# MARSLab-UMN/vi_depth_completion

Hardware: AMD Instinct MI355X
Metric: frames/sec (higher is better)
Workload: dtype f32

## Files before the change

### vi_depth_completion_amd/csrc/wfused.hip

```cpp
#include "common.h"
#include <cstdlib>

#pragma clang fp contract(off)

namespace {

typedef float f32x4 __attribute__((ext_vector_type(4)));

constexpr int TB = 16, NBW = 32, KC = 16, NPOS = 36;
constexpr int NPW = 8, NTW = 8, NTHREADS = 64 * (NPW + NTW);
constexpr int VBUF = NPOS * TB * KC;
constexpr int XSLOT = 37;
constexpr int XBUF = TB * XSLOT * KC;
constexpr int NDMA = TB * XSLOT / 16;
constexpr int MLD = 36;
constexpr size_t LDS_BYTES = (size_t)(2 * VBUF + 2 * XBUF) * sizeof(float);
static_assert(TB * XSLOT % 16 == 0, "whole DMA instructions");
static_assert((size_t)NPOS * TB * MLD * sizeof(float) <= LDS_BYTES, "the epilogue's product rows reuse the buffers");
static_assert(LDS_BYTES <= 160 * 1024, "one workgroup per CU");

struct FArgs {
    const float* x; const float* u; float* y; const float* s1; const float* b1; const float* s2; const float* b2;
    int H, W, Cin, ldx, Cout, ldy, th, tw, T, flags, nbn, gn;
    long long x_gs, w_gs, y_gs, p_gs;
    unsigned x_bytes;
};

typedef __attribute__((address_space(3))) void lds_void_t;

template <typename V> __device__ __forceinline__ void bt6_lo(const V (&d)[6], V (&t)[3]) {
    const V p = d[4] - 4.f * d[2], q = d[3] - 4.f * d[1];
    t[0] = (4.f * d[0] - 5.f * d[2]) + d[4];
    t[1] = p + q;
    t[2] = p - q;
}
template <typename V> __device__ __forceinline__ void bt6_hi(const V (&d)[6], V (&t)[3]) {
    const V r = d[4] - d[2], s = 2.f * (d[3] - d[1]);
    t[0] = r + s;
    t[1] = r - s;
    t[2] = (4.f * d[1] - 5.f * d[3]) + d[5];
}
template <typename V> __device__ __forceinline__ void bt6(const V (&d)[6], V (&t)[6]) {
    V lo[3], hi[3];
    bt6_lo(d, lo);
    bt6_hi(d, hi);
#pragma unroll
    for (int i = 0; i < 3; ++i) { t[i] = lo[i]; t[3 + i] = hi[i]; }
}
__device__ __forceinline__ void at6(const float (&m)[6], float (&o)[4]) {
    const float s12 = m[1] + m[2], d12 = m[1] - m[2], s34 = m[3] + m[4], d34 = m[3] - m[4];
    o[0] = (m[0] + s12) + s34;
    o[1] = d12 + 2.f * d34;
    o[2] = s12 + 4.f * s34;
    o[3] = (d12 + 8.f * d34) + m[5];
}

template <int N_> __device__ __forceinline__ void wait_lgkmcnt() { asm volatile("s_waitcnt lgkmcnt(%0)" ::"n"(N_) : "memory"); }
__device__ __forceinline__ f32x4 lds_read_b128(unsigned addr) {
    f32x4 v;
    asm volatile("ds_read_b128 %0, %1" : "=v"(v) : "v"(addr));
    return v;
}
template <int OFF> __device__ __forceinline__ float lds_read_b32(unsigned addr) {
    float v;
    asm volatile("ds_read_b32 %0, %1 offset:%2" : "=v"(v) : "v"(addr), "n"(OFF));
    return v;
}
template <int OFF> __device__ __forceinline__ void lds_write_b32(unsigned addr, float v) { asm volatile("ds_write_b32 %0, %1 offset:%2" ::"v"(addr), "v"(v), "n"(OFF) : "memory"); }

template <int PW, int NB, int DBG>
__device__ __forceinline__ void product_wave(const FArgs& a, float* smem, unsigned lds0, int lane, int pos0, int g, int nb, int NK) {
    const int n = lane & 15, kq = lane >> 4;
    const int n32 = a.Cout / 32, pair = NB == 2 ? nb : nb >> 1, half = NB == 2 ? 0 : nb & 1;
    const float* ub = a.u + (size_t)g * a.w_gs + ((size_t)pos0 * n32 + pair) * ((size_t)NK * 512) + half * 256 + lane * 4;
    const size_t pos_stride = (size_t)n32 * NK * 512;
    auto load_b = [&](int p, int kc, f32x4 (&dst)[NB]) {
        const float* s = ub + (size_t)p * pos_stride + (size_t)kc * 512;
        dst[0] = *reinterpret_cast<const f32x4*>(s);
        if constexpr (NB == 2) dst[1] = *reinterpret_cast<const f32x4*>(s + 256);
    };
    f32x4 acc[PW][NB];
#pragma unroll
    for (int p = 0; p < PW; ++p)
#pragma unroll
        for (int j = 0; j < NB; ++j) acc[p][j] = f32x4{0.f, 0.f, 0.f, 0.f};
    f32x4 bq[PW][NB];
#pragma unroll
    for (int p = 0; p < PW; ++p) load_b(p, 0, bq[p]);
    const unsigned a_off = (unsigned)((n * KC + ((kq ^ ((n >> 2) & 3)) * 4)) * 4);
    const unsigned a_wave = lds0 + (unsigned)(pos0 * TB * KC * 4);

    __builtin_amdgcn_s_barrier();
    __builtin_amdgcn_s_barrier();
    __builtin_amdgcn_s_barrier();
    for (int kc = 0; kc < NK; ++kc) {
        const unsigned vb = a_wave + (unsigned)((kc & 1) * VBUF * 4);
        const int kn = kc + 1 < NK ? kc + 1 : kc;
        f32x4 fa[2];
        fa[0] = lds_read_b128(vb + a_off);
#pragma unroll
        for (int p = 0; p < PW; ++p) {
            const int cur = p & 1, nxt = cur ^ 1;
            if (p + 1 < PW) {
                fa[nxt] = lds_read_b128(vb + (unsigned)((p + 1) * TB * KC * 4) + a_off);
                wait_lgkmcnt<1>();
            } else {
                wait_lgkmcnt<0>();
            }
            __builtin_amdgcn_sched_barrier(0);
#pragma unroll
            for (int ks = 0; ks < 4; ++ks)
#pragma unroll
                for (int j = 0; j < NB; ++j)
                    if constexpr (!(DBG & 1)) acc[p][j] = __builtin_amdgcn_mfma_f32_16x16x4f32(fa[cur][ks], bq[p][j][ks], acc[p][j], 0, 0, 0);
                    else if (ks == 0) acc[p][j][0] += fa[cur][0] + fa[cur][3] + bq[p][j][0] + bq[p][j][3];
            if constexpr (!(DBG & 2)) load_b(p, kn, bq[p]);
            __builtin_amdgcn_sched_barrier(0);
        }
        __builtin_amdgcn_s_barrier();
    }
    asm volatile("s_waitcnt vmcnt(0)" ::: "memory");
    float* mx = smem;
#pragma unroll
    for (int p = 0; p < PW; ++p)
#pragma unroll
        for (int j = 0; j < NB; ++j)
#pragma unroll
            for (int i = 0; i < 4; ++i) mx[((pos0 + p) * TB + 4 * kq + i) * MLD + j * 16 + n] = acc[p][j][i];
}

template <int NB, int DBG>
__global__ void __launch_bounds__(NTHREADS)
wino4_fused_kernel(const FArgs a) {
    extern __shared__ __attribute__((aligned(16))) float smem[];
    const int tid = threadIdx.x;
    const int L = blockIdx.x;
    const int tb = L / a.gn, r_ = L - tb * a.gn, g = r_ / a.nbn, nb = r_ - g * a.nbn;
    const int NK = a.Cin / KC;
    const unsigned lds0 = (unsigned)(size_t)((__attribute__((address_space(3))) float*)smem);

    if (tid < 64 * NPW) {
        const int w = __builtin_amdgcn_readfirstlane(tid >> 6);
        if (w < 4) product_wave<5, NB, DBG>(a, smem, lds0, tid & 63, 5 * w, g, nb, NK);
        else product_wave<4, NB, DBG>(a, smem, lds0, tid & 63, 20 + 4 * (w - 4), g, nb, NK);
    } else {
        const int tt = tid - 64 * NPW, lane = tid & 63;
        const int w8 = __builtin_amdgcn_readfirstlane(tt >> 6), grp = w8 >> 2;
        const int u_ = tt & 255, m = u_ >> 4, c = u_ & 15;
        const int tpf = a.th * a.tw;
        constexpr unsigned OOB = 0x80000000u;
        unsigned voff[5];
#pragma unroll
        for (int i = 0; i < 5; ++i) {
            const int j = w8 + 8 * i;
            const int slot = 16 * j + (lane >> 2), quad = lane & 3;
            const int ts = slot / XSLOT, px = slot - ts * XSLOT;
            const int t = tb * TB + ts;
            bool ok = j < NDMA && px < 36 && t < a.T;
            const int tc = ok ? t : 0;
            const int b = tc / tpf, rem = tc - b * tpf, ty = rem / a.tw, tx = rem - ty * a.tw;
            const int r = px / 6, s = px - r * 6;
            const int iy = ty * 4 - 1 + r, ix = tx * 4 - 1 + s;
            ok = ok && (unsigned)iy < (unsigned)a.H && (unsigned)ix < (unsigned)a.W;
            voff[i] = ok ? (unsigned)(((size_t)((b * a.H + iy) * a.W + ix) * a.ldx + (size_t)g * a.x_gs + quad * 4) * 4) : OOB;
        }
        const __amdgpu_buffer_rsrc_t x_rsrc = __builtin_amdgcn_make_buffer_rsrc(const_cast<float*>(a.x), 0, (int)a.x_bytes, 0x00020000);
        auto dma = [&](int cc) {
            float* dst = smem + 2 * VBUF + (cc & 1) * XBUF;
            const int soff = cc * KC * 4;
#pragma unroll
            for (int i = 0; i < 5; ++i)
                if (w8 + 8 * i < NDMA) __builtin_amdgcn_raw_ptr_buffer_load_lds(x_rsrc, (lds_void_t*)(dst + (w8 + 8 * i) * 256), 16, (int)voff[i], soff, 0, 0);
        };
        float out[36];
        const unsigned x_thr = lds0 + (unsigned)((2 * VBUF + (m * XSLOT) * KC + c) * 4);
        const unsigned v_thr = lds0 + (unsigned)((m * KC + (((c >> 2) ^ ((m >> 2) & 3)) * 4) + (c & 3)) * 4);
        auto phase_a = [&](int cc) {
            const unsigned xa = x_thr + (unsigned)((cc & 1) * XBUF * 4);
            float D[36];
#define VIDC_RD(i) D[i] = lds_read_b32<(i) * KC * 4>(xa);
            VIDC_RD(0) VIDC_RD(1) VIDC_RD(2) VIDC_RD(3) VIDC_RD(4) VIDC_RD(5) VIDC_RD(6) VIDC_RD(7) VIDC_RD(8) VIDC_RD(9) VIDC_RD(10) VIDC_RD(11)
            VIDC_RD(12) VIDC_RD(13) VIDC_RD(14) VIDC_RD(15) VIDC_RD(16) VIDC_RD(17) VIDC_RD(18) VIDC_RD(19) VIDC_RD(20) VIDC_RD(21) VIDC_RD(22) VIDC_RD(23)
            VIDC_RD(24) VIDC_RD(25) VIDC_RD(26) VIDC_RD(27) VIDC_RD(28) VIDC_RD(29) VIDC_RD(30) VIDC_RD(31) VIDC_RD(32) VIDC_RD(33) VIDC_RD(34) VIDC_RD(35)
#undef VIDC_RD
            asm volatile("s_waitcnt lgkmcnt(0)" : "+v"(D[0]), "+v"(D[1]), "+v"(D[2]), "+v"(D[3]), "+v"(D[4]), "+v"(D[5]), "+v"(D[6]), "+v"(D[7]), "+v"(D[8]), "+v"(D[9]), "+v"(D[10]), "+v"(D[11]), "+v"(D[12]), "+v"(D[13]), "+v"(D[14]), "+v"(D[15]), "+v"(D[16]), "+v"(D[17]) :: "memory");
            asm volatile("" : "+v"(D[18]), "+v"(D[19]), "+v"(D[20]), "+v"(D[21]), "+v"(D[22]), "+v"(D[23]), "+v"(D[24]), "+v"(D[25]), "+v"(D[26]), "+v"(D[27]), "+v"(D[28]), "+v"(D[29]), "+v"(D[30]), "+v"(D[31]), "+v"(D[32]), "+v"(D[33]), "+v"(D[34]), "+v"(D[35]) :: "memory");
            float tcol[6][6];
#pragma unroll
            for (int s = 0; s < 6; ++s) {
                float col[6], o6[6];
#pragma unroll
                for (int r = 0; r < 6; ++r) col[r] = D[r * 6 + s];
                bt6(col, o6);
#pragma unroll
                for (int r = 0; r < 6; ++r) tcol[r][s] = o6[r];
            }
#pragma unroll
            for (int r = 0; r < 6; ++r) {
                float o6[6];
                bt6(tcol[r], o6);
#pragma unroll
                for (int s = 0; s < 6; ++s) out[r * 6 + s] = o6[s];
            }
        };
        auto phase_b = [&](int cc) {
            const unsigned va = v_thr + (unsigned)((cc & 1) * VBUF * 4);
#define VIDC_WR(i) lds_write_b32<(i) * TB * KC * 4>(va, out[i]);
            VIDC_WR(0) VIDC_WR(1) VIDC_WR(2) VIDC_WR(3) VIDC_WR(4) VIDC_WR(5) VIDC_WR(6) VIDC_WR(7) VIDC_WR(8) VIDC_WR(9) VIDC_WR(10) VIDC_WR(11)
            VIDC_WR(12) VIDC_WR(13) VIDC_WR(14) VIDC_WR(15) VIDC_WR(16) VIDC_WR(17) VIDC_WR(18) VIDC_WR(19) VIDC_WR(20) VIDC_WR(21) VIDC_WR(22) VIDC_WR(23)
            VIDC_WR(24) VIDC_WR(25) VIDC_WR(26) VIDC_WR(27) VIDC_WR(28) VIDC_WR(29) VIDC_WR(30) VIDC_WR(31) VIDC_WR(32) VIDC_WR(33) VIDC_WR(34) VIDC_WR(35)
#undef VIDC_WR
        };
        auto fence_barrier = [&]() {
            if constexpr (DBG & 16) asm volatile("s_waitcnt lgkmcnt(0)" ::: "memory");
            else asm volatile("s_waitcnt vmcnt(0) lgkmcnt(0)" ::: "memory");
            __builtin_amdgcn_s_barrier();
        };
        dma(0);
        if (NK > 1) dma(1);
        fence_barrier();
        if (grp == 0) phase_a(0);
        else if (NK > 1) phase_a(1);
        fence_barrier();
        if (NK > 2) dma(2);
        if (grp == 0) phase_b(0);
        fence_barrier();
        for (int it = 0; it < NK; ++it) {
            if (!(DBG & 4)) {
                if (it + 3 < NK) dma(it + 3);
                if ((it & 1) == grp) {
                    if (it + 2 < NK) phase_a(it + 2);
                } else {
                    if (it + 1 < NK) phase_b(it + 1);
                }
            }
            fence_barrier();
        }
    }
    __syncthreads();
    if (tid < TB * 16 * NB) {
        const int m = tid / (16 * NB), c = tid - m * (16 * NB);
        const int t = tb * TB + m;
        if (t >= a.T || (DBG & 8)) return;
        const int tpf = a.th * a.tw;
        const int b = t / tpf, rem = t - b * tpf, ty = rem / a.tw, tx = rem - ty * a.tw;
        const float* mx = smem + m * MLD + c;
        float tc[4][6];
#pragma unroll
        for (int s = 0; s < 6; ++s) {
            float col[6], o4[4];
#pragma unroll
            for (int r = 0; r < 6; ++r) col[r] = mx[(r * 6 + s) * TB * MLD];
            at6(col, o4);
#pragma unroll
            for (int r = 0; r < 4; ++r) tc[r][s] = o4[r];
        }
        const int ch = nb * 16 * NB + c;
        const float s1 = a.s1[(size_t)g * a.p_gs + ch], b1 = a.b1[(size_t)g * a.p_gs + ch];
        const bool aff2 = a.flags & VIDC_AFFINE2;
        const float s2 = aff2 ? a.s2[(size_t)g * a.p_gs + ch] : 0.f, b2 = aff2 ? a.b2[(size_t)g * a.p_gs + ch] : 0.f;
        const float lo1 = (a.flags & VIDC_RELU1) ? 0.f : -INFINITY, lo2 = (a.flags & VIDC_RELU2) ? 0.f : -INFINITY;
        float* yb = a.y + (size_t)g * a.y_gs + ch;
#pragma unroll
        for (int r = 0; r < 4; ++r) {
            float o4[4];
            at6(tc[r], o4);
            const int oy = ty * 4 + r;
            if (oy >= a.H) continue;
#pragma unroll
            for (int s = 0; s < 4; ++s) {
                const int ox = tx * 4 + s;
                if (ox >= a.W) continue;
                float o = fmaxf(o4[s] * s1 + b1, lo1);
                if (aff2) o = fmaxf(o * s2 + b2, lo2);
                yb[((size_t)(b * a.H + oy) * a.W + ox) * a.ldy] = o;
            }
        }
    }
}

__global__ void __launch_bounds__(256)
wino4_pack_kernel(const float* __restrict__ u, float* __restrict__ o, int Cout, int Cin, long long total4) {
    const long long i = (long long)blockIdx.x * blockDim.x + threadIdx.x;
    if (i >= total4) return;
    const int NK = Cin / KC, nbn = Cout / NBW;
    const int lane = (int)(i & 63), nblk = (int)((i >> 6) & 1);
    long long r = i >> 7;
    const int kc = (int)(r % NK); r /= NK;
    const int nb = (int)(r % nbn);
    const int pos = (int)(r / nbn);
    const int n = lane & 15, kq = lane >> 4;
    const float4 v = *reinterpret_cast<const float4*>(u + ((size_t)pos * Cout + nb * NBW + nblk * 16 + n) * Cin + kc * KC + kq * 4);
    *reinterpret_cast<float4*>(o + i * 4) = v;
}

template <int NB, int DBG>
int launch_nb(const FArgs& a, long long wgs, hipStream_t st) {
    static bool attr_set[64] = {};
    int dev = 0;
    VIDC_HIP(hipGetDevice(&dev));
    if (dev < 0 || dev >= 64 || !attr_set[dev]) {
        VIDC_HIP(hipFuncSetAttribute(reinterpret_cast<const void*>(&wino4_fused_kernel<NB, DBG>), hipFuncAttributeMaxDynamicSharedMemorySize, (int)LDS_BYTES));
        if (dev >= 0 && dev < 64) attr_set[dev] = true;
    }
    hipLaunchKernelGGL((wino4_fused_kernel<NB, DBG>), dim3((unsigned)wgs), dim3(NTHREADS), LDS_BYTES, st, a);
    VIDC_CHECK_LAUNCH("wino4_fused_kernel");
    return VIDC_OK;
}

template <int DBG>
int launch_dbg(const FArgs& a, long long wgs, hipStream_t st) { return a.nbn * 32 == a.Cout ? launch_nb<2, DBG>(a, wgs, st) : launch_nb<1, DBG>(a, wgs, st); }

}

namespace vidc {

int launch_wino4_fused(const vidc_conv_desc& d, hipStream_t st) {
    VIDC_REQUIRE(d.precision == VIDC_PREC_FP32, VIDC_ERR_SHAPE, "conv (fused Winograd): fp32 arithmetic only");
    VIDC_REQUIRE(d.KH == 3 && d.KW == 3 && d.stride == 1 && d.pad == 1 && d.dilation <= 1, VIDC_ERR_SHAPE, "conv (fused Winograd): 3x3 / stride 1 / pad 1 / dense only");
    VIDC_REQUIRE(d.Cin % KC == 0 && d.Cout % NBW == 0 && d.ldx % 4 == 0, VIDC_ERR_SHAPE, "conv (fused Winograd): Cin %% 16 == 0, Cout %% 32 == 0, ldx %% 4 == 0");
    VIDC_REQUIRE(!(d.flags & ~(VIDC_RELU1 | VIDC_AFFINE2 | VIDC_RELU2)), VIDC_ERR_SHAPE, "conv (fused Winograd): flags 0x%x not supported (affine / ReLU / second affine / ReLU only)", d.flags);
    VIDC_REQUIRE(d.w_gs == (long long)NPOS * d.Cout * d.Cin || d.groups == 1, VIDC_ERR_SHAPE, "conv (fused Winograd): w = U of vidc_winograd_weight_pack_fused, w_gs = 36 * Cout * Cin");
    VIDC_REQUIRE((reinterpret_cast<uintptr_t>(d.x) & 15) == 0 && (reinterpret_cast<uintptr_t>(d.w) & 15) == 0 && d.x_gs % 4 == 0, VIDC_ERR_SHAPE, "conv (fused Winograd): x and U 16-byte aligned");
    FArgs a;
    a.x = d.x; a.u = d.w; a.y = d.y; a.s1 = d.scale1; a.b1 = d.shift1; a.s2 = d.scale2; a.b2 = d.shift2;
    a.H = d.H; a.W = d.W; a.Cin = d.Cin; a.ldx = d.ldx; a.Cout = d.Cout; a.ldy = d.ldy;
    a.th = (d.H + 3) / 4; a.tw = (d.W + 3) / 4;
    a.T = d.B * a.th * a.tw;
    static const int force_nb = [] { const char* e = getenv("VIDC_WFUSED_NB"); return e ? atoi(e) : 0; }();
    const long long wgs32 = (long long)((d.B * a.th * a.tw + TB - 1) / TB) * d.groups * (d.Cout / NBW);
    const int nbk = force_nb == 1 || force_nb == 2 ? force_nb : (wgs32 * 2 <= 256 ? 1 : 2);
    a.flags = d.flags; a.nbn = d.Cout / (16 * nbk); a.gn = d.groups * a.nbn;
    a.x_gs = d.x_gs; a.w_gs = d.w_gs; a.y_gs = d.y_gs; a.p_gs = d.p_gs;
    VIDC_REQUIRE((long long)d.B * d.H * d.W * d.ldx * 4 < (1ll << 30), VIDC_ERR_SHAPE, "conv (fused Winograd): the input must stay below 1 GiB");
    a.x_bytes = (unsigned)((long long)d.B * d.H * d.W * d.ldx * 4);
    const long long wgs = (long long)((a.T + TB - 1) / TB) * a.gn;
    VIDC_REQUIRE(wgs < (1ll << 31), VIDC_ERR_SHAPE, "conv (fused Winograd): grid too large");
#ifdef VIDC_WFUSED_ATTRIB
    static const int dbg = [] { const char* e = getenv("VIDC_WFUSED_DBG"); return e ? atoi(e) : 0; }();
    switch (dbg) {
        case 1: return launch_dbg<1>(a, wgs, st);
        case 2: return launch_dbg<2>(a, wgs, st);
        case 4: return launch_dbg<4>(a, wgs, st);
        case 8: return launch_dbg<8>(a, wgs, st);
        case 3: return launch_dbg<3>(a, wgs, st);
        case 6: return launch_dbg<6>(a, wgs, st);
        case 7: return launch_dbg<7>(a, wgs, st);
        case 15: return launch_dbg<15>(a, wgs, st);
        case 16: return launch_dbg<16>(a, wgs, st);
        default: break;
    }
#endif
    return launch_dbg<0>(a, wgs, st);
}

}

extern "C" int vidc_winograd_weight_pack_fused(const float* u, float* u_packed, int Cout, int Cin, vidc_stream_t stream) {
    VIDC_REQUIRE(u && u_packed && u != u_packed, VIDC_ERR_NULL, "vidc_winograd_weight_pack_fused: null pointer (or in place)");
    VIDC_REQUIRE(Cout > 0 && Cin > 0 && Cout % NBW == 0 && Cin % KC == 0, VIDC_ERR_SHAPE, "vidc_winograd_weight_pack_fused: Cout must be a multiple of 32, Cin of 16");
    const long long total4 = (long long)NPOS * Cout * Cin / 4;
    hipLaunchKernelGGL(wino4_pack_kernel, dim3((unsigned)((total4 + 255) / 256)), dim3(256), 0, vidc::as_stream(stream), u, u_packed, Cout, Cin, total4);
    VIDC_CHECK_LAUNCH("wino4_pack_kernel");
    return VIDC_OK;
}
```

Measured before the change: 635.3.

## Add persistent Winograd kernel specialised for Cin=64 convolutions

Adds a persistent-grid Winograd F(4,3) kernel used whenever Cin is 64. Each workgroup holds all 64 input channels' weights in registers and keeps them across work items that share the same output-channel block. It prefetches the next tile's input patch during the epilogue and uses buffer loads and stores for bounds handling. The goal is to avoid reloading weights per tile and to cut launch/grid overhead for these layers. In exchange it raises register pressure and ties the grid size to the CU count.

```diff
diff --git a/vi_depth_completion_amd/csrc/wfused.hip b/vi_depth_completion_amd/csrc/wfused.hip
--- a/vi_depth_completion_amd/csrc/wfused.hip
+++ b/vi_depth_completion_amd/csrc/wfused.hip
@@ -24,6 +24,8 @@
     int H, W, Cin, ldx, Cout, ldy, th, tw, T, flags, nbn, gn;
     long long x_gs, w_gs, y_gs, p_gs;
     unsigned x_bytes;
+    int items;
+    unsigned y_bytes;
 };
 
 typedef __attribute__((address_space(3))) void lds_void_t;
@@ -279,6 +281,169 @@
     }
 }
 
+constexpr int SK = 64, SNK = SK / KC, SWAVES = 8, STHREADS = 64 * SWAVES, SPW = NPOS * 2 / SWAVES;
+constexpr int SVB = NPOS * SNK * TB * KC;
+constexpr size_t S_LDS_BYTES = (size_t)SVB * sizeof(float);
+static_assert(SPW * SWAVES == NPOS * 2, "whole positions per wave");
+static_assert(NPOS * TB * MLD <= SVB, "the product rows reuse V");
+static_assert(S_LDS_BYTES <= 160 * 1024, "one workgroup per CU");
+static_assert(STHREADS == TB * NBW, "fold: one thread per (tile, channel)");
+static_assert(SNK * (TB / 4) == 2 * SWAVES, "transform: two passes of (chunk, four tiles) per wave");
+
+template <int DBG>
+__global__ void __launch_bounds__(STHREADS)
+wino4_stem_kernel(const FArgs a) {
+    extern __shared__ __attribute__((aligned(16))) float smem[];
+    const int tid = threadIdx.x, lane = tid & 63;
+    const int w = __builtin_amdgcn_readfirstlane(tid >> 6);
+    const int nwg = (int)gridDim.x;
+    int L = (int)blockIdx.x;
+    if ((nwg & 7) == 0) L = (L & 7) * (nwg >> 3) + (L >> 3);
+    const int n32 = a.nbn, tpf = a.th * a.tw;
+    const int n = lane & 15, kq = lane >> 4;
+    const int jb = w & 1, pos0 = SPW * (w >> 1);
+    constexpr unsigned OOB_ROW = 0x80000000u, OOB_COL = 0x40000000u;
+    const __amdgpu_buffer_rsrc_t x_rsrc = __builtin_amdgcn_make_buffer_rsrc(const_cast<float*>(a.x), 0, (int)a.x_bytes, 0x00020000);
+    const __amdgpu_buffer_rsrc_t y_rsrc = __builtin_amdgcn_make_buffer_rsrc(a.y, 0, (int)a.y_bytes, 0x00020000);
+    const int a_off = n * KC + ((kq ^ ((n >> 2) & 3)) * 4);
+    auto load_patch = [&](int tb, int g, int pass, float (&D)[36]) {
+        const int q = pass * SWAVES + w, kc = q & 3, m = (q >> 2) * 4 + (lane >> 4), c16 = lane & 15;
+        const int t = tb * TB + m;
+        const bool tok = t < a.T;
+        const int tc = tok ? t : 0;
+        const int b = tc / tpf, rem = tc - b * tpf, ty = rem / a.tw, tx = rem - ty * a.tw;
+        unsigned rowo[6], colo[6];
+#pragma unroll
+        for (int r = 0; r < 6; ++r) {
+            const int iy = ty * 4 - 1 + r, ix = tx * 4 - 1 + r;
+            rowo[r] = tok && (unsigned)iy < (unsigned)a.H ? (unsigned)((b * a.H + iy) * a.W) * (unsigned)a.ldx * 4u : OOB_ROW;
+            colo[r] = (unsigned)ix < (unsigned)a.W ? (unsigned)(((size_t)ix * a.ldx + (size_t)g * a.x_gs + kc * KC + c16) * 4) : OOB_COL;
+        }
+#pragma unroll
+        for (int r = 0; r < 6; ++r)
+#pragma unroll
+            for (int s = 0; s < 6; ++s)
+                if constexpr (!(DBG & 2)) D[r * 6 + s] = __builtin_bit_cast(float, __builtin_amdgcn_raw_buffer_load_b32(x_rsrc, (int)(rowo[r] + colo[s]), 0, 0));
+                else D[r * 6 + s] = __builtin_bit_cast(float, rowo[r] + colo[s]);
+    };
+    auto col_step = [&](const float (&D)[36], float (&tcol)[6][6]) {
+#pragma unroll
+        for (int s = 0; s < 6; ++s) {
+            float col[6], o6[6];
+#pragma unroll
+            for (int r = 0; r < 6; ++r) col[r] = D[r * 6 + s];
+            bt6(col, o6);
+#pragma unroll
+            for (int r = 0; r < 6; ++r) tcol[r][s] = o6[r];
+        }
+    };
+    auto row_step = [&](const float (&tcol)[6][6], int pass) {
+        const int q = pass * SWAVES + w, kc = q & 3, m = (q >> 2) * 4 + (lane >> 4), c16 = lane & 15;
+        float* vw = smem + (kc * TB + m) * KC + (((c16 >> 2) ^ ((m >> 2) & 3)) * 4) + (c16 & 3);
+#pragma unroll
+        for (int r = 0; r < 6; ++r) {
+            float o6[6];
+            bt6(tcol[r], o6);
+#pragma unroll
+            for (int s = 0; s < 6; ++s) vw[(r * 6 + s) * (SNK * TB * KC)] = o6[s];
+        }
+    };
+    const int fm = tid >> 5, fc = tid & 31;
+    f32x4 U[SPW][SNK];
+    float s1 = 0.f, b1 = 0.f, s2 = 0.f, b2 = 0.f;
+    const bool aff2 = a.flags & VIDC_AFFINE2;
+    const float lo1 = (a.flags & VIDC_RELU1) ? 0.f : -INFINITY, lo2 = (a.flags & VIDC_RELU2) ? 0.f : -INFINITY;
+    int cur = -1;
+    float D[36];
+    if constexpr (!(DBG & 4))
+        if (L < a.items) load_patch(L / a.gn, (L % a.gn) / n32, 0, D);
+    for (int item = L; item < a.items; item += nwg) {
+        const int tb = item / a.gn, combo = item - tb * a.gn, g = combo / n32, pair = combo - g * n32;
+        if (combo != cur) {
+            cur = combo;
+            const float* ub = a.u + (size_t)g * a.w_gs + ((size_t)pos0 * n32 + pair) * (size_t)(SNK * 512) + jb * 256 + lane * 4;
+#pragma unroll
+            for (int u = 0; u < SPW; ++u)
+#pragma unroll
+                for (int kc = 0; kc < SNK; ++kc) U[u][kc] = *reinterpret_cast<const f32x4*>(ub + (size_t)u * n32 * (SNK * 512) + kc * 512);
+            const size_t pc = (size_t)g * a.p_gs + pair * NBW + fc;
+            s1 = a.s1[pc]; b1 = a.b1[pc];
+            if (aff2) { s2 = a.s2[pc]; b2 = a.b2[pc]; }
+        }
+        if constexpr (!(DBG & 4)) {
+            float tcol[6][6];
+            col_step(D, tcol);
+            load_patch(tb, g, 1, D);
+            row_step(tcol, 0);
+            col_step(D, tcol);
+            row_step(tcol, 1);
+        }
+        __syncthreads();
+        f32x4 acc[SPW];
+#pragma unroll
+        for (int u = 0; u < SPW; ++u) acc[u] = f32x4{0.f, 0.f, 0.f, 0.f};
+        const float* va = smem + pos0 * (SNK * TB * KC) + a_off;
+#pragma unroll
+        for (int kc = 0; kc < SNK; ++kc) {
+            f32x4 fa[SPW];
+#pragma unroll
+            for (int u = 0; u < SPW; ++u) fa[u] = *reinterpret_cast<const f32x4*>(va + (u * SNK + kc) * (TB * KC));
+#pragma unroll
+            for (int ks = 0; ks < 4; ++ks)
+#pragma unroll
+                for (int u = 0; u < SPW; ++u)
+                    if constexpr (!(DBG & 1)) acc[u] = __builtin_amdgcn_mfma_f32_16x16x4f32(fa[u][ks], U[u][kc][ks], acc[u], 0, 0, 0);
+                    else if (ks == 0) acc[u][0] += fa[u][0] + fa[u][3] + U[u][kc][0] + U[u][kc][3];
+        }
+        __syncthreads();
+#pragma unroll
+        for (int u = 0; u < SPW; ++u)
+#pragma unroll
+            for (int i = 0; i < 4; ++i) smem[((pos0 + u) * TB + 4 * kq + i) * MLD + jb * 16 + n] = acc[u][i];
+        __syncthreads();
+        if constexpr (!(DBG & 4)) {
+            const int nxt = item + nwg < a.items ? item + nwg : item;
+            load_patch(nxt / a.gn, (nxt % a.gn) / n32, 0, D);
+        }
+        if constexpr (!(DBG & 8)) {
+            const int t = tb * TB + fm;
+            const bool tok = t < a.T;
+            const int tc = tok ? t : 0;
+            const int b = tc / tpf, rem = tc - b * tpf, ty = rem / a.tw, tx = rem - ty * a.tw;
+            unsigned rowo[4], colo[4];
+#pragma unroll
+            for (int r = 0; r < 4; ++r) {
+                const int oy = ty * 4 + r, ox = tx * 4 + r;
+                rowo[r] = tok && oy < a.H ? (unsigned)((b * a.H + oy) * a.W) * (unsigned)a.ldy * 4u : OOB_ROW;
+                colo[r] = ox < a.W ? (unsigned)(((size_t)ox * a.ldy + (size_t)g * a.y_gs + pair * NBW + fc) * 4) : OOB_COL;
+            }
+            const float* mx = smem + fm * MLD + fc;
+            float tc4[4][6];
+#pragma unroll
+            for (int s = 0; s < 6; ++s) {
+                float col[6], o4[4];
+#pragma unroll
+                for (int r = 0; r < 6; ++r) col[r] = mx[(r * 6 + s) * TB * MLD];
+                at6(col, o4);
+#pragma unroll
+                for (int r = 0; r < 4; ++r) tc4[r][s] = o4[r];
+            }
+#pragma unroll
+            for (int r = 0; r < 4; ++r) {
+                float o4[4];
+                at6(tc4[r], o4);
+#pragma unroll
+                for (int s = 0; s < 4; ++s) {
+                    float o = fmaxf(o4[s] * s1 + b1, lo1);
+                    if (aff2) o = fmaxf(o * s2 + b2, lo2);
+                    __builtin_amdgcn_raw_buffer_store_b32(__builtin_bit_cast(unsigned, o), y_rsrc, (int)(rowo[r] + colo[s]), 0, 0);
+                }
+            }
+        }
+        __syncthreads();
+    }
+}
+
 __global__ void __launch_bounds__(256)
 wino4_pack_kernel(const float* __restrict__ u, float* __restrict__ o, int Cout, int Cin, long long total4) {
     const long long i = (long long)blockIdx.x * blockDim.x + threadIdx.x;
@@ -310,6 +475,59 @@
 
 template <int DBG>
 int launch_dbg(const FArgs& a, long long wgs, hipStream_t st) { return a.nbn * 32 == a.Cout ? launch_nb<2, DBG>(a, wgs, st) : launch_nb<1, DBG>(a, wgs, st); }
+
+template <int DBG>
+int launch_stem_dbg(const FArgs& a, long long wgs, hipStream_t st) {
+    static bool attr_set[64] = {};
+    int dev = 0;
+    VIDC_HIP(hipGetDevice(&dev));
+    if (dev < 0 || dev >= 64 || !attr_set[dev]) {
+        VIDC_HIP(hipFuncSetAttribute(reinterpret_cast<const void*>(&wino4_stem_kernel<DBG>), hipFuncAttributeMaxDynamicSharedMemorySize, (int)S_LDS_BYTES));
+        if (dev >= 0 && dev < 64) attr_set[dev] = true;
+    }
+    hipLaunchKernelGGL(wino4_stem_kernel<DBG>, dim3((unsigned)wgs), dim3(STHREADS), S_LDS_BYTES, st, a);
+    VIDC_CHECK_LAUNCH("wino4_stem_kernel");
+    return VIDC_OK;
+}
+
+int launch_stem(FArgs& a, const vidc_conv_desc& d, hipStream_t st) {
+    static int n_cu[64] = {};
+    int dev = 0;
+    VIDC_HIP(hipGetDevice(&dev));
+    const bool cached = dev >= 0 && dev < 64;
+    int cus = cached ? n_cu[dev] : 0;
+    if (cus <= 0) {
+        VIDC_HIP(hipDeviceGetAttribute(&cus, hipDeviceAttributeMultiprocessorCount, dev));
+        VIDC_REQUIRE(cus > 0, VIDC_ERR_SHAPE, "conv (fused Winograd): no compute units");
+        if (cached) n_cu[dev] = cus;
+    }
+    a.nbn = d.Cout / NBW; a.gn = d.groups * a.nbn;
+    const long long y_bytes = ((long long)(d.groups - 1) * d.y_gs + ((long long)d.B * d.H * d.W - 1) * d.ldy + d.Cout) * 4;
+    VIDC_REQUIRE(d.y_gs >= 0 && d.ldy > 0 && y_bytes < (1ll << 30), VIDC_ERR_SHAPE, "conv (fused Winograd, Cin = 64): the output must stay below 1 GiB");
+    a.y_bytes = (unsigned)y_bytes;
+    const long long items = (long long)((a.T + TB - 1) / TB) * a.gn;
+    VIDC_REQUIRE(items > 0 && items < (1ll << 30), VIDC_ERR_SHAPE, "conv (fused Winograd): grid too large");
+    a.items = (int)items;
+    const char* e = getenv("VIDC_WFUSED_WGS");
+    const int forced = e ? atoi(e) : 0;
+    long long wgs = forced > 0 ? forced : (a.gn <= cus ? (long long)(cus / a.gn) * a.gn : cus);
+    if (wgs > items) wgs = items;
+#ifdef VIDC_WFUSED_ATTRIB
+    static const int dbg = [] { const char* v = getenv("VIDC_WFUSED_DBG"); return v ? atoi(v) : 0; }();
+    switch (dbg) {
+        case 1: return launch_stem_dbg<1>(a, wgs, st);
+        case 2: return launch_stem_dbg<2>(a, wgs, st);
+        case 4: return launch_stem_dbg<4>(a, wgs, st);
+        case 8: return launch_stem_dbg<8>(a, wgs, st);
+        case 3: return launch_stem_dbg<3>(a, wgs, st);
+        case 5: return launch_stem_dbg<5>(a, wgs, st);
+        case 12: return launch_stem_dbg<12>(a, wgs, st);
+        case 13: return launch_stem_dbg<13>(a, wgs, st);
+        default: break;
+    }
+#endif
+    return launch_stem_dbg<0>(a, wgs, st);
+}
 
 }
 
@@ -334,7 +552,9 @@
     a.x_gs = d.x_gs; a.w_gs = d.w_gs; a.y_gs = d.y_gs; a.p_gs = d.p_gs;
     VIDC_REQUIRE((long long)d.B * d.H * d.W * d.ldx * 4 < (1ll << 30), VIDC_ERR_SHAPE, "conv (fused Winograd): the input must stay below 1 GiB");
     a.x_bytes = (unsigned)((long long)d.B * d.H * d.W * d.ldx * 4);
-    const long long wgs = (long long)((a.T + TB - 1) / TB) * a.gn;
+    a.items = 0;
+    if (d.Cin == SK) return launch_stem(a, d, st);
+    const long long wgs =(long long)((a.T + TB - 1) / TB) * a.gn;
     VIDC_REQUIRE(wgs < (1ll << 31), VIDC_ERR_SHAPE, "conv (fused Winograd): grid too large");
 #ifdef VIDC_WFUSED_ATTRIB
     static const int dbg = [] { const char* e = getenv("VIDC_WFUSED_DBG"); return e ? atoi(e) : 0; }();
```

Result: no change. 636.0 (median of 2 runs) (+0.1%).

## Add persistent Winograd stem kernel for Cin=64 with register-held accumulators

Applied to the files above, without the earlier changes.

Adds a persistent-grid fused Winograd F(4,3) kernel used when Cin is 64 and the tile count is large. Each workgroup loops over several tile/channel items with 4 product waves and 4 transform waves. The product waves keep all 36 position accumulators in registers across the four K-chunks, stream weights from global memory through a 6-deep register ring, and run the output transform and affine/ReLU epilogue directly from registers with vectorized 16-byte stores. This targets launch overhead, weight staging through LDS and the LDS round-trip in the epilogue. In exchange it raises register pressure and reduces per-CU parallelism, since the grid is capped at the CU count.

```diff
diff --git a/vi_depth_completion_amd/csrc/wfused.hip b/vi_depth_completion_amd/csrc/wfused.hip
--- a/vi_depth_completion_amd/csrc/wfused.hip
+++ b/vi_depth_completion_amd/csrc/wfused.hip
@@ -1,4 +1,5 @@
 #include "common.h"
+#include <cstdio>
 #include <cstdlib>
 
 #pragma clang fp contract(off)
@@ -279,6 +280,222 @@
     }
 }
 
+constexpr int SNK = 4;
+constexpr int SNPW = 4, SNTW = 4, STHREADS = 64 * (SNPW + SNTW);
+constexpr int SRING = 6;
+constexpr int SDMA = (NDMA + SNTW - 1) / SNTW;
+static_assert(NPOS % SRING == 0 && SRING % 2 == 0, "the ring slot of a position is a compile-time constant");
+
+template <int DBG>
+__device__ __forceinline__ void stem_product_wave(const FArgs& a, unsigned lds0, int lane, int w, int S) {
+    const int n = lane & 15, kq = lane >> 4;
+    const int n32 = a.Cout / 32;
+    const size_t pos_stride = (size_t)n32 * SNK * 512;
+    auto step_ptr = [&](int q) -> const float* {
+        const int I = (int)blockIdx.x + (q >> 2) * (int)gridDim.x;
+        const int r_ = I % a.gn, g = r_ / a.nbn, h = r_ - g * a.nbn;
+        const int nb16 = h * 4 + w;
+        return a.u + (size_t)g * a.w_gs + (size_t)(nb16 >> 1) * (SNK * 512) + (nb16 & 1) * 256 + lane * 4 + (q & 3) * 512;
+    };
+    f32x4 acc[NPOS];
+#pragma unroll
+    for (int p = 0; p < NPOS; ++p) acc[p] = f32x4{0.f, 0.f, 0.f, 0.f};
+    const float* cur = step_ptr(0);
+    f32x4 bq[SRING];
+#pragma unroll
+    for (int e = 0; e < SRING; ++e) bq[e] = *reinterpret_cast<const f32x4*>(cur + (size_t)e * pos_stride);
+    const unsigned a_off = lds0 + (unsigned)((n * KC + ((kq ^ ((n >> 2) & 3)) * 4)) * 4);
+
+    __builtin_amdgcn_s_barrier();
+    __builtin_amdgcn_s_barrier();
+    for (int q = 0; q < S; ++q) {
+        const float* nxt = step_ptr(q + 1 < S ? q + 1 : q);
+        const unsigned vb = a_off + (unsigned)((q & 1) * VBUF * 4);
+        f32x4 fa[2][2];
+        fa[0][0] = lds_read_b128(vb);
+        fa[0][1] = lds_read_b128(vb + (unsigned)(TB * KC * 4));
+#pragma unroll
+        for (int j = 0; j < NPOS / 2; ++j) {
+            const int c = j & 1, x = c ^ 1, p0 = 2 * j;
+            if (j + 1 < NPOS / 2) {
+                fa[x][0] = lds_read_b128(vb + (unsigned)((p0 + 2) * TB * KC * 4));
+                fa[x][1] = lds_read_b128(vb + (unsigned)((p0 + 3) * TB * KC * 4));
+                wait_lgkmcnt<2>();
+            } else {
+                wait_lgkmcnt<0>();
+            }
+            __builtin_amdgcn_sched_barrier(0);
+#pragma unroll
+            for (int ks = 0; ks < 4; ++ks) {
+                if constexpr (!(DBG & 1)) {
+                    acc[p0] = __builtin_amdgcn_mfma_f32_16x16x4f32(bq[p0 % SRING][ks], fa[c][0][ks], acc[p0], 0, 0, 0);
+                    acc[p0 + 1] = __builtin_amdgcn_mfma_f32_16x16x4f32(bq[(p0 + 1) % SRING][ks], fa[c][1][ks], acc[p0 + 1], 0, 0, 0);
+                } else if (ks == 0) {
+                    acc[p0][0] += fa[c][0][0] + fa[c][0][3] + bq[p0 % SRING][0] + bq[p0 % SRING][3];
+                    acc[p0 + 1][0] += fa[c][1][0] + fa[c][1][3] + bq[(p0 + 1) % SRING][0] + bq[(p0 + 1) % SRING][3];
+                }
+            }
+            if constexpr (!(DBG & 2)) {
+                const int pn = p0 + SRING;
+                const float* s = pn < NPOS ? cur + (size_t)pn * pos_stride : nxt + (size_t)(pn - NPOS) * pos_stride;
+                bq[p0 % SRING] = *reinterpret_cast<const f32x4*>(s);
+                bq[(p0 + 1) % SRING] = *reinterpret_cast<const f32x4*>(s + pos_stride);
+            }
+            __builtin_amdgcn_sched_barrier(0);
+        }
+        __builtin_amdgcn_s_barrier();
+        cur = nxt;
+        if ((q & 3) != 3) continue;
+        if (!(DBG & 8) || a.H < 0) {
+            const int I = (int)blockIdx.x + (q >> 2) * (int)gridDim.x;
+            const int tb = I / a.gn, r_ = I - tb * a.gn, g = r_ / a.nbn, h = r_ - g * a.nbn;
+            const int ch = h * 64 + w * 16 + 4 * kq;
+            const bool aff2 = a.flags & VIDC_AFFINE2;
+            const size_t pof = (size_t)g * a.p_gs + ch;
+            const float lo1 = (a.flags & VIDC_RELU1) ? 0.f : -INFINITY, lo2 = (a.flags & VIDC_RELU2) ? 0.f : -INFINITY;
+            const int tpf = a.th * a.tw;
+            const int t = tb * TB + n, tcl = t < a.T ? t : 0;
+            const int b = tcl / tpf, rem = tcl - b * tpf, ty = rem / a.tw, tx = rem - ty * a.tw;
+            const bool okt = t < a.T && (!(DBG & 16) || a.H < 0);
+            float* yb = a.y + (size_t)g * a.y_gs + ch + ((size_t)(b * a.H + ty * 4) * a.W + tx * 4) * a.ldy;
+            float tc[4][4][6];
+#pragma unroll
+            for (int s = 0; s < 6; ++s) {
+#pragma unroll
+                for (int i = 0; i < 4; ++i) {
+                    float col[6], o4[4];
+#pragma unroll
+                    for (int r = 0; r < 6; ++r) col[r] = acc[r * 6 + s][i];
+                    at6(col, o4);
+#pragma unroll
+                    for (int r = 0; r < 4; ++r) tc[i][r][s] = o4[r];
+                }
+                __builtin_amdgcn_sched_barrier(0);
+            }
+            const f32x4 s1 = *reinterpret_cast<const f32x4*>(a.s1 + pof), b1 = *reinterpret_cast<const f32x4*>(a.b1 + pof);
+            const f32x4 s2 = *reinterpret_cast<const f32x4*>((aff2 ? a.s2 : a.s1) + pof), b2 = *reinterpret_cast<const f32x4*>((aff2 ? a.b2 : a.b1) + pof);
+#pragma unroll
+            for (int r = 0; r < 4; ++r) {
+                float o[4][4];
+#pragma unroll
+                for (int i = 0; i < 4; ++i) {
+                    at6(tc[i][r], o[i]);
+#pragma unroll
+                    for (int s = 0; s < 4; ++s) {
+                        float v = fmaxf(o[i][s] * s1[i] + b1[i], lo1);
+                        if (aff2) v = fmaxf(v * s2[i] + b2[i], lo2);
+                        o[i][s] = v;
+                    }
+                }
+#pragma unroll
+                for (int s = 0; s < 4; ++s)
+                    if (okt && ty * 4 + r < a.H && tx * 4 + s < a.W)
+                        *reinterpret_cast<f32x4*>(yb + ((size_t)r * a.W + s) * a.ldy) = f32x4{o[0][s], o[1][s], o[2][s], o[3][s]};
+            }
+        }
+#pragma unroll
+        for (int p = 0; p < NPOS; ++p) acc[p] = f32x4{0.f, 0.f, 0.f, 0.f};
+    }
+}
+
+template <int DBG>
+__global__ void __launch_bounds__(STHREADS)
+wino4_fused_stem_kernel(const FArgs a, const int nitems) {
+    extern __shared__ __attribute__((aligned(16))) float smem[];
+    const int tid = threadIdx.x;
+    const int S = SNK * ((nitems - 1 - (int)blockIdx.x) / (int)gridDim.x + 1);
+    const unsigned lds0 = (unsigned)(size_t)((__attribute__((address_space(3))) float*)smem);
+
+    if (tid < 64 * SNPW) {
+        stem_product_wave<DBG>(a, lds0, tid & 63, __builtin_amdgcn_readfirstlane(tid >> 6), S);
+        return;
+    }
+    const int tt = tid - 64 * SNPW, lane = tid & 63;
+    const int w4 = __builtin_amdgcn_readfirstlane(tt >> 6);
+    const int m = tt >> 4, c = tt & 15;
+    const int tpf = a.th * a.tw;
+    constexpr unsigned OOB = 0x80000000u;
+    unsigned voff[SDMA];
+    auto item_offsets = [&](int I) {
+        const int tb = I / a.gn, r_ = I - tb * a.gn, g = r_ / a.nbn;
+#pragma unroll
+        for (int i = 0; i < SDMA; ++i) {
+            const int j = w4 + SNTW * i;
+            const int slot = 16 * j + (lane >> 2), quad = lane & 3;
+            const int ts = slot / XSLOT, px = slot - ts * XSLOT;
+            const int t = tb * TB + ts;
+            bool ok = j < NDMA && px < 36 && t < a.T;
+            const int tc = ok ? t : 0;
+            const int b = tc / tpf, rem = tc - b * tpf, ty = rem / a.tw, tx = rem - ty * a.tw;
+            const int r = px / 6, s = px - r * 6;
+            const int iy = ty * 4 - 1 + r, ix = tx * 4 - 1 + s;
+            ok = ok && (unsigned)iy < (unsigned)a.H && (unsigned)ix < (unsigned)a.W;
+            voff[i] = ok ? (unsigned)(((size_t)((b * a.H + iy) * a.W + ix) * a.ldx + (size_t)g * a.x_gs + quad * 4) * 4) : OOB;
+        }
+    };
+    const __amdgpu_buffer_rsrc_t x_rsrc = __builtin_amdgcn_make_buffer_rsrc(const_cast<float*>(a.x), 0, (int)a.x_bytes, 0x00020000);
+    auto dma = [&](int q) {
+        if ((q & 3) == 0) item_offsets((int)blockIdx.x + (q >> 2) * (int)gridDim.x);
+        float* dst = smem + 2 * VBUF + (q & 1) * XBUF;
+        const int soff = (q & 3) * KC * 4;
+#pragma unroll
+        for (int i = 0; i < SDMA; ++i)
+            if (w4 + SNTW * i < NDMA) __builtin_amdgcn_raw_ptr_buffer_load_lds(x_rsrc, (lds_void_t*)(dst + (w4 + SNTW * i) * 256), 16, (int)voff[i], soff, 0, 0);
+    };
+    const unsigned x_thr = lds0 + (unsigned)((2 * VBUF + (m * XSLOT) * KC + c) * 4);
+    const unsigned v_thr = lds0 + (unsigned)((m * KC + (((c >> 2) ^ ((m >> 2) & 3)) * 4) + (c & 3)) * 4);
+    auto transform = [&](int q) {
+        const unsigned xa = x_thr + (unsigned)((q & 1) * XBUF * 4);
+        float D[36], out[36];
+#define VIDC_RD(i) D[i] = lds_read_b32<(i) * KC * 4>(xa);
+        VIDC_RD(0) VIDC_RD(1) VIDC_RD(2) VIDC_RD(3) VIDC_RD(4) VIDC_RD(5) VIDC_RD(6) VIDC_RD(7) VIDC_RD(8) VIDC_RD(9) VIDC_RD(10) VIDC_RD(11)
+        VIDC_RD(12) VIDC_RD(13) VIDC_RD(14) VIDC_RD(15) VIDC_RD(16) VIDC_RD(17) VIDC_RD(18) VIDC_RD(19) VIDC_RD(20) VIDC_RD(21) VIDC_RD(22) VIDC_RD(23)
+        VIDC_RD(24) VIDC_RD(25) VIDC_RD(26) VIDC_RD(27) VIDC_RD(28) VIDC_RD(29) VIDC_RD(30) VIDC_RD(31) VIDC_RD(32) VIDC_RD(33) VIDC_RD(34) VIDC_RD(35)
+#undef VIDC_RD
+        asm volatile("s_waitcnt lgkmcnt(0)" : "+v"(D[0]), "+v"(D[1]), "+v"(D[2]), "+v"(D[3]), "+v"(D[4]), "+v"(D[5]), "+v"(D[6]), "+v"(D[7]), "+v"(D[8]), "+v"(D[9]), "+v"(D[10]), "+v"(D[11]), "+v"(D[12]), "+v"(D[13]), "+v"(D[14]), "+v"(D[15]), "+v"(D[16]), "+v"(D[17]) :: "memory");
+        asm volatile("" : "+v"(D[18]), "+v"(D[19]), "+v"(D[20]), "+v"(D[21]), "+v"(D[22]), "+v"(D[23]), "+v"(D[24]), "+v"(D[25]), "+v"(D[26]), "+v"(D[27]), "+v"(D[28]), "+v"(D[29]), "+v"(D[30]), "+v"(D[31]), "+v"(D[32]), "+v"(D[33]), "+v"(D[34]), "+v"(D[35]) :: "memory");
+        float tcol[6][6];
+#pragma unroll
+        for (int s = 0; s < 6; ++s) {
+            float col[6], o6[6];
+#pragma unroll
+            for (int r = 0; r < 6; ++r) col[r] = D[r * 6 + s];
+            bt6(col, o6);
+#pragma unroll
+            for (int r = 0; r < 6; ++r) tcol[r][s] = o6[r];
+        }
+#pragma unroll
+        for (int r = 0; r < 6; ++r) {
+            float o6[6];
+            bt6(tcol[r], o6);
+#pragma unroll
+            for (int s = 0; s < 6; ++s) out[r * 6 + s] = o6[s];
+        }
+        const unsigned va = v_thr + (unsigned)((q & 1) * VBUF * 4);
+#define VIDC_WR(i) lds_write_b32<(i) * TB * KC * 4>(va, out[i]);
+        VIDC_WR(0) VIDC_WR(1) VIDC_WR(2) VIDC_WR(3) VIDC_WR(4) VIDC_WR(5) VIDC_WR(6) VIDC_WR(7) VIDC_WR(8) VIDC_WR(9) VIDC_WR(10) VIDC_WR(11)
+        VIDC_WR(12) VIDC_WR(13) VIDC_WR(14) VIDC_WR(15) VIDC_WR(16) VIDC_WR(17) VIDC_WR(18) VIDC_WR(19) VIDC_WR(20) VIDC_WR(21) VIDC_WR(22) VIDC_WR(23)
+        VIDC_WR(24) VIDC_WR(25) VIDC_WR(26) VIDC_WR(27) VIDC_WR(28) VIDC_WR(29) VIDC_WR(30) VIDC_WR(31) VIDC_WR(32) VIDC_WR(33) VIDC_WR(34) VIDC_WR(35)
+#undef VIDC_WR
+    };
+    auto fence_barrier = [&]() {
+        asm volatile("s_waitcnt vmcnt(0) lgkmcnt(0)" ::: "memory");
+        __builtin_amdgcn_s_barrier();
+    };
+    dma(0);
+    dma(1);
+    fence_barrier();
+    transform(0);
+    fence_barrier();
+    for (int q = 0; q < S; ++q) {
+        if (!(DBG & 4)) {
+            if (q + 2 < S) dma(q + 2);
+            if (q + 1 < S) transform(q + 1);
+        }
+        fence_barrier();
+    }
+}
+
 __global__ void __launch_bounds__(256)
 wino4_pack_kernel(const float* __restrict__ u, float* __restrict__ o, int Cout, int Cin, long long total4) {
     const long long i = (long long)blockIdx.x * blockDim.x + threadIdx.x;
@@ -305,6 +522,34 @@
     }
     hipLaunchKernelGGL((wino4_fused_kernel<NB, DBG>), dim3((unsigned)wgs), dim3(NTHREADS), LDS_BYTES, st, a);
     VIDC_CHECK_LAUNCH("wino4_fused_kernel");
+    return VIDC_OK;
+}
+
+template <int DBG>
+int launch_stem(FArgs& a, int groups, hipStream_t st) {
+    static bool attr_set[64] = {};
+    static int cus[64] = {};
+    int dev = 0;
+    VIDC_HIP(hipGetDevice(&dev));
+    const bool cached = dev >= 0 && dev < 64;
+    if (!cached || !attr_set[dev]) {
+        VIDC_HIP(hipFuncSetAttribute(reinterpret_cast<const void*>(&wino4_fused_stem_kernel<DBG>), hipFuncAttributeMaxDynamicSharedMemorySize, (int)LDS_BYTES));
+        if (cached) attr_set[dev] = true;
+    }
+    int ncu = cached ? cus[dev] : 0;
+    if (ncu <= 0) {
+        VIDC_HIP(hipDeviceGetAttribute(&ncu, hipDeviceAttributeMultiprocessorCount, dev));
+        if (ncu <= 0) ncu = 256;
+        if (cached) cus[dev] = ncu;
+    }
+    a.nbn = a.Cout / 64; a.gn = groups * a.nbn;
+    const long long items = (long long)((a.T + TB - 1) / TB) * a.gn;
+    VIDC_REQUIRE(items * SNK < (1ll << 31), VIDC_ERR_SHAPE, "conv (fused Winograd): grid too large");
+    long long cap = ncu;
+    if (const char* e = getenv("VIDC_WFUSED_STEM_CAP")) { const long long v = atoll(e); if (v > 0) cap = v; }
+    const long long wgs = items < cap ? items : cap;
+    hipLaunchKernelGGL((wino4_fused_stem_kernel<DBG>), dim3((unsigned)wgs), dim3(STHREADS), LDS_BYTES, st, a, (int)items);
+    VIDC_CHECK_LAUNCH("wino4_fused_stem_kernel");
     return VIDC_OK;
 }
 
@@ -334,6 +579,33 @@
     a.x_gs = d.x_gs; a.w_gs = d.w_gs; a.y_gs = d.y_gs; a.p_gs = d.p_gs;
     VIDC_REQUIRE((long long)d.B * d.H * d.W * d.ldx * 4 < (1ll << 30), VIDC_ERR_SHAPE, "conv (fused Winograd): the input must stay below 1 GiB");
     a.x_bytes = (unsigned)((long long)d.B * d.H * d.W * d.ldx * 4);
+    {
+        long long min_tiles = 4096;
+        if (const char* e = getenv("VIDC_WFUSED_STEM_MIN_TILES")) { const long long v = atoll(e); min_tiles = v > 0 ? v : (1ll << 62); }
+        auto al16 = [](const void* p) { return (reinterpret_cast<uintptr_t>(p) & 15) == 0; };
+        const bool y16 = al16(d.y) && d.ldy % 4 == 0 && d.y_gs % 4 == 0 && d.p_gs % 4 == 0 && al16(d.scale1) && al16(d.shift1) &&
+                         (!(d.flags & VIDC_AFFINE2) || (al16(d.scale2) && al16(d.shift2)));
+        const bool stem = d.Cin == 64 && d.Cout % 64 == 0 && y16 && (long long)a.T * d.groups * (d.Cout / 64) >= min_tiles;
+        if (const char* e = getenv("VIDC_WFUSED_TRACE")) if (atoi(e)) fprintf(stderr, "wino4f: form %s Cin %d Cout %d tiles %d groups %d\n", stem ? "stem" : "4", d.Cin, d.Cout, a.T, d.groups);
+        if (stem) {
+#ifdef VIDC_WFUSED_ATTRIB
+            static const int sdbg = [] { const char* e = getenv("VIDC_WFUSED_DBG"); return e ? atoi(e) : 0; }();
+            switch (sdbg) {
+                case 1: return launch_stem<1>(a, d.groups, st);
+                case 2: return launch_stem<2>(a, d.groups, st);
+                case 4: return launch_stem<4>(a, d.groups, st);
+                case 8: return launch_stem<8>(a, d.groups, st);
+                case 3: return launch_stem<3>(a, d.groups, st);
+                case 7: return launch_stem<7>(a, d.groups, st);
+                case 10: return launch_stem<10>(a, d.groups, st);
+                case 15: return launch_stem<15>(a, d.groups, st);
+                case 16: return launch_stem<16>(a, d.groups, st);
+                default: break;
+            }
+#endif
+            return launch_stem<0>(a, d.groups, st);
+        }
+    }
     const long long wgs = (long long)((a.T + TB - 1) / TB) * a.gn;
     VIDC_REQUIRE(wgs < (1ll << 31), VIDC_ERR_SHAPE, "conv (fused Winograd): grid too large");
 #ifdef VIDC_WFUSED_ATTRIB
```

Result: faster. 631.3 before, 647.6 after (median of 6 runs) (+2.6%).
